# google-research/multinerf

Measured on NVIDIA H100. Metric: train-step rays/sec @16384 rays x (64+64+32) samples, higher is better.
Workload: dtype bf16

## Files before the change

multinerf_b200/csrc/chain.cu:

```cuda
#include <stdlib.h>
#include <string.h>

#include <algorithm>

#include "tc_common.cuh"

namespace mnrf {

constexpr int CH_W = 256;
constexpr int CH_ROWS = 128;
constexpr int CH_KBLK = CH_ROWS * 128;
constexpr int CH_WBLK = CH_W * 128;
constexpr int CH_SLOT = CH_WBLK + CH_KBLK;
constexpr int CH_SLOTS = 3;
constexpr int CH_ACT = 4 * CH_KBLK;
constexpr int CH_THREADS = 384;
constexpr int CH_MAX_LAYERS = MNRF_CHAIN_MAX_LAYERS;
constexpr int CH_SMEM = CH_ACT + CH_SLOTS * CH_SLOT + CH_MAX_LAYERS * CH_W * 4  + 256  +
                        1024 ;
static_assert(CH_SMEM <= 232448, "shared memory budget");

struct alignas(64) ChainMaps {
  CUtensorMap stream;
  CUtensorMap w[CH_MAX_LAYERS];
  CUtensorMap out[CH_MAX_LAYERS];
};

struct ChainLayer {
  int n_stream, stream_col0, stream_kb0;
  int n_res, res_kb0;
  int store;
  const float* bias;
  uint32_t* maskbits;
  int64_t ldmaskbits;
  float* colsum;
};

struct ChainParams {
  int num_layers;
  int64_t m;
  int64_t num_units;
  ChainLayer layer[CH_MAX_LAYERS];
  const float* head_w;
  const float* head_b;
  float* head_out;
};

__device__ __forceinline__ uint32_t pack_bf16_relu(float lo, float hi) {
  uint32_t r;
  asm("cvt.rn.relu.bf16x2.f32 %0, %1, %2;" : "=r"(r) : "f"(hi), "f"(lo));
  return r;
}

template <int MODE, int NH>
__global__ void __launch_bounds__(CH_THREADS, 1)
mlp_chain_kernel(const __grid_constant__ ChainMaps maps, const ChainParams p) {
  extern __shared__ uint8_t smem_dyn[];
  uint8_t* smem = reinterpret_cast<uint8_t*>((reinterpret_cast<uintptr_t>(smem_dyn) + 1023) & ~uintptr_t(1023));
  uint8_t* act = smem;
  uint8_t* ring = smem + CH_ACT;
  float* cs_s = reinterpret_cast<float*>(ring + CH_SLOTS * CH_SLOT);
  uint64_t* full_bar = reinterpret_cast<uint64_t*>(cs_s + CH_MAX_LAYERS * CH_W);
  uint64_t* empty_bar = full_bar + CH_SLOTS;

  const int warp = threadIdx.x >> 5;
  const int lane = threadIdx.x & 31;
  const int wg = threadIdx.x >> 7;

  if (threadIdx.x == 0) {
    bool any_stream = false;
    for (int j = 0; j < p.num_layers; ++j) {
      prefetch_tmap(&maps.w[j]);
      if (p.layer[j].store) prefetch_tmap(&maps.out[j]);
      any_stream |= p.layer[j].n_stream > 0;
    }
    if (any_stream) prefetch_tmap(&maps.stream);
    for (int i = 0; i < CH_SLOTS; ++i) { mbar_init(&full_bar[i], 1); mbar_init(&empty_bar[i], 8); }
    fence_barrier_init();
  }
  if (MODE == 1)
    for (int i = threadIdx.x; i < CH_MAX_LAYERS * CH_W; i += CH_THREADS) cs_s[i] = 0.f;
  __syncthreads();
  pdl_launch_dependents();
  pdl_wait();

  if (wg == 0) {
    setmaxnreg_dec<40>();
    if (threadIdx.x == 0) {
      uint32_t slot = 0, phase = 0;
      for (int64_t unit = blockIdx.x; unit < p.num_units; unit += gridDim.x) {
        const int row0 = (int)(unit * CH_ROWS);
        for (int j = 0; j < p.num_layers; ++j) {
          const ChainLayer& L = p.layer[j];
          for (int s = 0; s < L.n_res + L.n_stream; ++s) {
            const bool streamed = s >= L.n_res;
            const int si = s - L.n_res;
            mbar_wait(&empty_bar[slot], phase ^ 1, 1);
            mbar_expect_tx(&full_bar[slot], streamed ? CH_SLOT : CH_WBLK);
            uint8_t* sl = ring + slot * CH_SLOT;
            const int kb = streamed ? L.stream_kb0 + si : L.res_kb0 + s;
            tma_load_2d(sl, &maps.w[j], &full_bar[slot], kb * 64, 0);
            if (streamed) tma_load_2d(sl + CH_WBLK, &maps.stream, &full_bar[slot], L.stream_col0 + si * 64, row0);
            if (++slot == CH_SLOTS) { slot = 0; phase ^= 1; }
          }
        }
      }
    }
  } else {
    setmaxnreg_inc<232>();
    const int c = wg - 1;
    const int w = warp & 3;
    const int r_in = 64 * c + 16 * w + (lane >> 2);
    const int cq = 2 * (lane & 3);
    const uint32_t ring_s = smem_u32(ring), act_s = smem_u32(act);
    const bool lead = (threadIdx.x & 127) == 0;
    uint32_t slot = 0, phase = 0;
    float acc[CH_W / 2];
    for (int64_t unit = blockIdx.x; unit < p.num_units; unit += gridDim.x) {
      for (int j = 0; j < p.num_layers; ++j) {
        const ChainLayer& L = p.layer[j];
        const bool last = (j == p.num_layers - 1);
        const bool do_head = (MODE == 0) && last && p.head_w != nullptr;
        int prev = -1;
        fence_acc(acc);
        for (int s = 0; s < L.n_res + L.n_stream; ++s) {
          const bool streamed = s >= L.n_res;
          mbar_wait(&full_bar[slot], phase, 3);
          const uint32_t sl = ring_s + slot * CH_SLOT;
          const uint32_t a0 = (streamed ? sl + CH_WBLK : act_s + s * CH_KBLK) + c * (64 * 128);
          wgmma_fence();
#pragma unroll
          for (int k = 0; k < 64 / WGMMA_K; ++k)
            Wgmma<CH_W, 0, 0>::mma(acc, make_smem_desc(a0 + k * (WGMMA_K * 2), 0, 1024),
                                   make_smem_desc(sl + k * (WGMMA_K * 2), 0, 1024), (s > 0 || k > 0) ? 1u : 0u);
          wgmma_commit();
          wgmma_wait<1>();
          if (prev >= 0 && lane == 0) mbar_arrive(&empty_bar[prev]);
          prev = (int)slot;
          if (++slot == CH_SLOTS) { slot = 0; phase ^= 1; }
        }
        wgmma_wait<0>();
        fence_acc(acc);
        if (prev >= 0 && lane == 0) mbar_arrive(&empty_bar[prev]);

        if (lead) tma_store_wait_read<0>();
        named_bar_sync(1 + c, 128);
        int64_t rows[2];
        bool row_ok[2];
#pragma unroll
        for (int h = 0; h < 2; ++h) {
          rows[h] = unit * CH_ROWS + r_in + 8 * h;
          row_ok[h] = rows[h] < p.m;
        }
        uint32_t bits[2] = {0u, 0u};
        float hdot[NH][2];
#pragma unroll
        for (int o = 0; o < NH; ++o) hdot[o][0] = hdot[o][1] = 0.f;
#pragma unroll
        for (int i = 0; i < CH_W / 8; ++i) {
          const int col = 8 * i + cq;
          float v[2][2];
#pragma unroll
          for (int h = 0; h < 2; ++h) { v[h][0] = acc[4 * i + 2 * h]; v[h][1] = acc[4 * i + 2 * h + 1]; }
          uint32_t o[2];
          if (MODE == 0) {
            const float2 b = __ldg(reinterpret_cast<const float2*>(L.bias + col));
#pragma unroll
            for (int h = 0; h < 2; ++h) {
              v[h][0] += b.x;
              v[h][1] += b.y;
              bits[h] |= ((v[h][0] > 0.f ? 1u : 0u) | (v[h][1] > 0.f ? 2u : 0u)) << (col & 31);
              o[h] = pack_bf16_relu(v[h][0], v[h][1]);
            }
            if (do_head) {
#pragma unroll
              for (int oo = 0; oo < NH; ++oo) {
                const float2 hw = __ldg(reinterpret_cast<const float2*>(p.head_w + oo * CH_W + col));
#pragma unroll
                for (int h = 0; h < 2; ++h) hdot[oo][h] += bf16_lo(o[h]) * hw.x + bf16_hi(o[h]) * hw.y;
              }
            }
          } else {
#pragma unroll
            for (int h = 0; h < 2; ++h) {
              if (L.maskbits) {
                const uint32_t wd = row_ok[h] ? __ldg(L.maskbits + rows[h] * L.ldmaskbits + (col >> 5)) : 0u;
                if (!((wd >> (col & 31)) & 1u)) v[h][0] = 0.f;
                if (!((wd >> ((col + 1) & 31)) & 1u)) v[h][1] = 0.f;
              }
              o[h] = pack_bf16(v[h][0], v[h][1]);
            }
            if (L.colsum) {
              float s0 = v[0][0] + v[1][0], s1 = v[0][1] + v[1][1];
#pragma unroll
              for (int sh = 4; sh < 32; sh <<= 1) {
                s0 += __shfl_xor_sync(0xffffffffu, s0, sh);
                s1 += __shfl_xor_sync(0xffffffffu, s1, sh);
              }
              if (lane < 4) { atomicAdd(cs_s + j * CH_W + col, s0); atomicAdd(cs_s + j * CH_W + col + 1, s1); }
            }
          }
#pragma unroll
          for (int h = 0; h < 2; ++h) {
            const int r = r_in + 8 * h;
            st_shared_u32(act_s + (col >> 6) * CH_KBLK + r * 128 + ((((col & 63) >> 3) ^ (r & 7)) << 4) + (cq << 1), o[h]);
          }
          if (MODE == 0 && (i & 3) == 3) {
#pragma unroll
            for (int h = 0; h < 2; ++h) {
              bits[h] |= __shfl_xor_sync(0xffffffffu, bits[h], 1);
              bits[h] |= __shfl_xor_sync(0xffffffffu, bits[h], 2);
              if (L.maskbits && row_ok[h] && (lane & 3) == ((i >> 2) & 3))
                L.maskbits[rows[h] * L.ldmaskbits + (col >> 5)] = bits[h];
              bits[h] = 0u;
            }
          }
        }
        fence_proxy_async();
        named_bar_sync(1 + c, 128);
        if (lead && L.store) {
#pragma unroll
          for (int kb = 0; kb < 4; ++kb)
            tma_store_2d(&maps.out[j], act + kb * CH_KBLK + c * (64 * 128), kb * 64, (int)(unit * CH_ROWS) + 64 * c);
          tma_store_commit();
        }
        if (do_head) {
#pragma unroll
          for (int oo = 0; oo < NH; ++oo)
#pragma unroll
            for (int h = 0; h < 2; ++h) {
              hdot[oo][h] += __shfl_xor_sync(0xffffffffu, hdot[oo][h], 1);
              hdot[oo][h] += __shfl_xor_sync(0xffffffffu, hdot[oo][h], 2);
              if ((lane & 3) == 0 && row_ok[h])
                p.head_out[rows[h] * NH + oo] = hdot[oo][h] + (p.head_b ? __ldg(p.head_b + oo) : 0.f);
            }
        }
      }
    }
    if (lead) tma_store_wait_all();
    if (MODE == 1) {
      named_bar_sync(3, 256);
      for (int jj = 0; jj < p.num_layers; ++jj) {
        if (!p.layer[jj].colsum) continue;
        for (int i = threadIdx.x - 128; i < CH_W; i += 256) atomicAdd(p.layer[jj].colsum + i, cs_s[jj * CH_W + i]);
      }
    }
  }
}

}

extern "C" int mnrf_mlp_chain_max_layers(void) { return mnrf::CH_MAX_LAYERS; }

extern "C" int mnrf_mlp_chain(const mnrf_chain_desc* d, mnrf_stream stream_) {
  using namespace mnrf;
  cudaStream_t stream = (cudaStream_t)stream_;
  MNRF_CHECK(d, "mnrf_mlp_chain: null descriptor");
  if (d->m == 0) return 0;
  MNRF_CHECK(d->mode == MNRF_CHAIN_FWD || d->mode == MNRF_CHAIN_BWD, "mnrf_mlp_chain: bad mode %d", d->mode);
  MNRF_CHECK(d->num_layers >= 1 && d->num_layers <= CH_MAX_LAYERS, "mnrf_mlp_chain: 1..%d layers, got %d",
             CH_MAX_LAYERS, d->num_layers);
  MNRF_CHECK(d->width == CH_W, "mnrf_mlp_chain: layer width must be %d, got %d", CH_W, d->width);
  const int sms = mnrf_num_sms();
  ChainMaps maps;
  memset(&maps, 0, sizeof(maps));
  ChainParams p{};
  p.num_layers = d->num_layers;
  p.m = d->m;
  p.num_units = (d->m + CH_ROWS - 1) / CH_ROWS;
  bool any_stream = false;
  for (int j = 0; j < d->num_layers; ++j) {
    const mnrf_chain_layer& s = d->layer[j];
    ChainLayer& L = p.layer[j];
    MNRF_CHECK(s.n_res == 0 || s.n_res == CH_W / 64, "mnrf_mlp_chain: layer %d: n_res must be 0 or %d", j, CH_W / 64);
    MNRF_CHECK(s.n_stream >= 0 && (s.n_stream > 0 || s.n_res > 0), "mnrf_mlp_chain: layer %d has no operand", j);
    MNRF_CHECK(j > 0 || s.n_res == 0, "mnrf_mlp_chain: the first layer has no resident operand");
    MNRF_CHECK(s.w && ((uintptr_t)s.w % 16) == 0 && s.ldw % 8 == 0, "mnrf_mlp_chain: layer %d: weights must be 16-byte aligned", j);
    const int kblocks = std::max(s.n_stream > 0 ? s.stream_kb0 + s.n_stream : 0, s.n_res > 0 ? s.res_kb0 + s.n_res : 0);
    MNRF_CHECK(s.ldw >= (int64_t)kblocks * 64, "mnrf_mlp_chain: layer %d: weight pitch %lld < K %d", j, (long long)s.ldw, kblocks * 64);
    L.n_stream = s.n_stream; L.stream_col0 = s.stream_col0; L.stream_kb0 = s.stream_kb0;
    L.n_res = s.n_res; L.res_kb0 = s.res_kb0;
    L.store = s.out ? 1 : 0;
    L.bias = s.bias; L.maskbits = s.maskbits; L.ldmaskbits = s.ldmaskbits; L.colsum = s.colsum;
    if (s.bias) MNRF_CHECK(((uintptr_t)s.bias % 8) == 0, "mnrf_mlp_chain: layer %d: bias must be 8-byte aligned", j);
    if (s.maskbits)
      MNRF_CHECK(s.ldmaskbits >= CH_W / 32, "mnrf_mlp_chain: layer %d: maskbits rows must hold >= %d words", j, CH_W / 32);
    if (d->mode == MNRF_CHAIN_BWD) MNRF_CHECK(!s.bias, "mnrf_mlp_chain: bias is a forward input");
    else MNRF_CHECK(s.bias && !s.colsum, "mnrf_mlp_chain: layer %d: the forward chain takes a bias and no colsum", j);
    if (make_tmap(&maps.w[j], s.w, CH_W, (int64_t)kblocks * 64, s.ldw, 64, CH_W)) return 1;
    if (s.out) {
      MNRF_CHECK(((uintptr_t)s.out % 16) == 0 && s.ldo % 8 == 0 && s.ldo >= CH_W, "mnrf_mlp_chain: layer %d: output alignment", j);
      if (make_tmap(&maps.out[j], s.out, d->m, CH_W, s.ldo, 64, 64)) return 1;
    }
    any_stream |= s.n_stream > 0;
    if (s.n_stream > 0)
      MNRF_CHECK(s.stream_col0 % 64 == 0 && s.stream_col0 + s.n_stream * 64 <= d->stream_cols,
                 "mnrf_mlp_chain: layer %d: streamed columns [%d, %d) outside the stream tensor (%d columns)", j,
                 s.stream_col0, s.stream_col0 + s.n_stream * 64, d->stream_cols);
  }
  if (any_stream) {
    MNRF_CHECK(d->stream && ((uintptr_t)d->stream % 16) == 0 && d->ldstream % 8 == 0 && d->stream_cols % 64 == 0,
               "mnrf_mlp_chain: streamed operand must be 16-byte aligned with a multiple of 64 columns");
    if (make_tmap(&maps.stream, d->stream, d->m, d->stream_cols, d->ldstream, 64, CH_ROWS)) return 1;
  }
  p.head_w = d->head_w; p.head_b = d->head_b; p.head_out = d->head_out;
  const int head_n = d->head_n ? d->head_n : 1;
  if (d->head_w) MNRF_CHECK(d->mode == MNRF_CHAIN_FWD && d->head_out && ((uintptr_t)d->head_w % 16) == 0,
                            "mnrf_mlp_chain: the head is a forward output (16-byte aligned weights)");
  MNRF_CHECK(head_n == 1 || (head_n == 4 && d->head_w), "mnrf_mlp_chain: head_n must be 1 or 4, got %d", head_n);
  cudaLaunchConfig_t cfg = {};
  cfg.gridDim = dim3((unsigned)std::min<int64_t>(p.num_units, sms)); cfg.blockDim = dim3(CH_THREADS);
  cfg.dynamicSmemBytes = CH_SMEM; cfg.stream = stream;
  cudaLaunchAttribute attr[1];
  attr[0].id = cudaLaunchAttributeProgrammaticStreamSerialization;
  attr[0].val.programmaticStreamSerializationAllowed = 1;
  cfg.attrs = attr; cfg.numAttrs = pdl_enabled() ? 1 : 0;
  if (d->mode == MNRF_CHAIN_FWD && head_n == 4) {
    static bool set4 = false;
    auto kern = mlp_chain_kernel<0, 4>;
    if (!set4) { MNRF_CUDA(cudaFuncSetAttribute(kern, cudaFuncAttributeMaxDynamicSharedMemorySize, CH_SMEM)); set4 = true; }
    MNRF_CUDA(cudaLaunchKernelEx(&cfg, kern, maps, p));
  } else if (d->mode == MNRF_CHAIN_FWD) {
    static bool set0 = false;
    auto kern = mlp_chain_kernel<0, 1>;
    if (!set0) { MNRF_CUDA(cudaFuncSetAttribute(kern, cudaFuncAttributeMaxDynamicSharedMemorySize, CH_SMEM)); set0 = true; }
    MNRF_CUDA(cudaLaunchKernelEx(&cfg, kern, maps, p));
  } else {
    static bool set1 = false;
    auto kern = mlp_chain_kernel<1, 1>;
    if (!set1) { MNRF_CUDA(cudaFuncSetAttribute(kern, cudaFuncAttributeMaxDynamicSharedMemorySize, CH_SMEM)); set1 = true; }
    MNRF_CUDA(cudaLaunchKernelEx(&cfg, kern, maps, p));
  }
  MNRF_LAUNCH_CHECK();
  return 0;
}
```

Measured before the change: 187,100.

## Split chain MLP into N-halves to overlap epilogue with next wgmma

Each layer's 256-wide output is split into two 128-column halves, each with its own accumulator. The hi half's MMAs and the next layer's lead-in are issued while the lo half's epilogue runs, so tensor-core work overlaps the bias/ReLU/mask epilogue. The ring now holds single-operand stages (7 of them), and the activations are triple-buffered across 6 blocks. Streamed inputs are reloaded for each half, which doubles their TMA traffic. A clock-based stuck detector that traps on deadlock is also added.

```diff
diff --git a/multinerf_b200/csrc/chain.cu b/multinerf_b200/csrc/chain.cu
--- a/multinerf_b200/csrc/chain.cu
+++ b/multinerf_b200/csrc/chain.cu
@@ -8,17 +8,19 @@
 namespace mnrf {
 
 constexpr int CH_W = 256;
+constexpr int CH_HALF = CH_W / 2;
 constexpr int CH_ROWS = 128;
 constexpr int CH_KBLK = CH_ROWS * 128;
-constexpr int CH_WBLK = CH_W * 128;
-constexpr int CH_SLOT = CH_WBLK + CH_KBLK;
-constexpr int CH_SLOTS = 3;
-constexpr int CH_ACT = 4 * CH_KBLK;
+constexpr int CH_STAGE = CH_HALF * 128;
+static_assert(CH_STAGE == CH_KBLK, "a ring stage holds either operand");
+constexpr int CH_STAGES = 7;
+constexpr int CH_ACT_BUFS = 6;
 constexpr int CH_THREADS = 384;
 constexpr int CH_MAX_LAYERS = MNRF_CHAIN_MAX_LAYERS;
-constexpr int CH_SMEM = CH_ACT + CH_SLOTS * CH_SLOT + CH_MAX_LAYERS * CH_W * 4  + 256  +
-                        1024 ;
+constexpr int CH_SMEM = CH_ACT_BUFS * CH_KBLK + CH_STAGES * CH_STAGE + CH_MAX_LAYERS * CH_W * 4  +
+                        256  + 1024 ;
 static_assert(CH_SMEM <= 232448, "shared memory budget");
+static_assert(2 * CH_STAGES * 8 <= 256, "barrier space");
 
 struct alignas(64) ChainMaps {
   CUtensorMap stream;
@@ -52,16 +54,198 @@
   return r;
 }
 
+struct ChainRing {
+  uint32_t ring_s;
+  uint64_t* full_bar;
+  uint64_t* empty_bar;
+  uint32_t iss, rel;
+  bool stuck;
+
+  __device__ __forceinline__ uint32_t take() {
+    const uint32_t st = iss++;
+    uint64_t* bar = &full_bar[st % CH_STAGES];
+    const uint32_t parity = (st / CH_STAGES) & 1u;
+    if (!mbar_try_wait(bar, parity)) {
+      const long long t0 = clock64();
+      while (!stuck && !mbar_try_wait(bar, parity)) stuck = clock64() - t0 > 4000000000LL;
+    }
+    return ring_s + (st % CH_STAGES) * CH_STAGE;
+  }
+  __device__ __forceinline__ void release(uint32_t upto, int lane) {
+    for (; rel < upto; ++rel)
+      if (lane == 0) mbar_arrive(&empty_bar[rel % CH_STAGES]);
+  }
+};
+
+__device__ __forceinline__ void chain_issue(float (&acc)[64], const ChainLayer& L, int q0, int q1, ChainRing& R,
+                                            uint32_t act_s, int prev, int c) {
+  for (int q = q0; q < q1; ++q) {
+    uint32_t a0;
+    if (q < L.n_res) a0 = act_s + ((prev + q) % CH_ACT_BUFS) * CH_KBLK;
+    else a0 = R.take();
+    a0 += c * (64 * 128);
+    const uint32_t w0 = R.take();
+    wgmma_fence();
+#pragma unroll
+    for (int k = 0; k < 64 / WGMMA_K; ++k)
+      Wgmma<CH_HALF, 0, 0>::mma(acc, make_smem_desc(a0 + k * (WGMMA_K * 2), 0, 1024),
+                                make_smem_desc(w0 + k * (WGMMA_K * 2), 0, 1024), (q > 0 || k > 0) ? 1u : 0u);
+  }
+}
+
+__device__ __forceinline__ void chain_rest(float (&acc)[64], const ChainLayer& L, int q0, ChainRing& R,
+                                           uint32_t act_s, int prev, int c, int lane) {
+  for (int q = q0; q < L.n_res + L.n_stream; ++q) {
+    const uint32_t first = R.iss;
+    chain_issue(acc, L, q, q + 1, R, act_s, prev, c);
+    wgmma_commit();
+    wgmma_wait<1>();
+    R.release(first, lane);
+  }
+}
+
+__device__ __forceinline__ int chain_fit(const ChainLayer& L, int cap, const ChainRing& R) {
+  int room = CH_STAGES - (int)(R.iss - R.rel), n = 0;
+  for (; n < cap && n < L.n_res + L.n_stream; ++n) {
+    room -= n < L.n_res ? 1 : 2;
+    if (room < 0) break;
+  }
+  return n;
+}
+
+__device__ __forceinline__ void chain_lead_in(float (&acc)[64], const ChainLayer& L, int n, ChainRing& R,
+                                              uint32_t act_s, int prev, int c, int lane) {
+  const uint32_t first = R.iss;
+  fence_acc(acc);
+  chain_issue(acc, L, 0, n, R, act_s, prev, c);
+  wgmma_commit();
+  wgmma_wait<1>();
+  R.release(first, lane);
+}
+
+struct ChainRows {
+  int64_t unit;
+  int64_t rows[2];
+  bool row_ok[2];
+};
+
+template <int MODE, int NH, int H>
+__device__ __forceinline__ void chain_epilogue(const float (&acc)[64], const ChainParams& p, const ChainMaps& maps,
+                                               int j, const ChainRows& rw, float (&hdot)[NH][2], uint32_t act_s,
+                                               uint8_t* act, int cur, float* cs_s, int c, int r_in, int cq,
+                                               int lane, bool lead) {
+  const ChainLayer& L = p.layer[j];
+  const bool do_head = (MODE == 0) && j == p.num_layers - 1 && p.head_w != nullptr;
+  const int b0 = (cur + 2 * H) % CH_ACT_BUFS, b1 = (cur + 2 * H + 1) % CH_ACT_BUFS;
+  uint32_t mw[2][4];
+  if (MODE == 1) {
+#pragma unroll
+    for (int h = 0; h < 2; ++h)
+#pragma unroll
+      for (int wd = 0; wd < 4; ++wd)
+        mw[h][wd] = L.maskbits && rw.row_ok[h] ? __ldg(L.maskbits + rw.rows[h] * L.ldmaskbits + 4 * H + wd) : 0u;
+  }
+  if (lead) tma_store_wait_read<2>();
+  named_bar_sync(1 + c, 128);
+  uint32_t bits[2] = {0u, 0u};
+  if (H == 0) {
+#pragma unroll
+    for (int o = 0; o < NH; ++o) hdot[o][0] = hdot[o][1] = 0.f;
+  }
+#pragma unroll
+  for (int i = 0; i < CH_HALF / 8; ++i) {
+    const int col = CH_HALF * H + 8 * i + cq;
+    float v[2][2];
+#pragma unroll
+    for (int h = 0; h < 2; ++h) { v[h][0] = acc[4 * i + 2 * h]; v[h][1] = acc[4 * i + 2 * h + 1]; }
+    uint32_t o[2];
+    if (MODE == 0) {
+      const float2 b = __ldg(reinterpret_cast<const float2*>(L.bias + col));
+#pragma unroll
+      for (int h = 0; h < 2; ++h) {
+        v[h][0] += b.x;
+        v[h][1] += b.y;
+        bits[h] |= ((v[h][0] > 0.f ? 1u : 0u) | (v[h][1] > 0.f ? 2u : 0u)) << (col & 31);
+        o[h] = pack_bf16_relu(v[h][0], v[h][1]);
+      }
+      if (do_head) {
+#pragma unroll
+        for (int oo = 0; oo < NH; ++oo) {
+          const float2 hw = __ldg(reinterpret_cast<const float2*>(p.head_w + oo * CH_W + col));
+#pragma unroll
+          for (int h = 0; h < 2; ++h) hdot[oo][h] += bf16_lo(o[h]) * hw.x + bf16_hi(o[h]) * hw.y;
+        }
+      }
+    } else {
+#pragma unroll
+      for (int h = 0; h < 2; ++h) {
+        if (L.maskbits) {
+          const uint32_t wd = mw[h][i >> 2];
+          if (!((wd >> (col & 31)) & 1u)) v[h][0] = 0.f;
+          if (!((wd >> ((col + 1) & 31)) & 1u)) v[h][1] = 0.f;
+        }
+        o[h] = pack_bf16(v[h][0], v[h][1]);
+      }
+      if (L.colsum) {
+        float s0 = v[0][0] + v[1][0], s1 = v[0][1] + v[1][1];
+#pragma unroll
+        for (int sh = 4; sh < 32; sh <<= 1) {
+          s0 += __shfl_xor_sync(0xffffffffu, s0, sh);
+          s1 += __shfl_xor_sync(0xffffffffu, s1, sh);
+        }
+        if (lane < 4) { atomicAdd(cs_s + j * CH_W + col, s0); atomicAdd(cs_s + j * CH_W + col + 1, s1); }
+      }
+    }
+    const uint32_t blk = act_s + (i < 8 ? b0 : b1) * CH_KBLK;
+#pragma unroll
+    for (int h = 0; h < 2; ++h) {
+      const int r = r_in + 8 * h;
+      st_shared_u32(blk + r * 128 + ((((col & 63) >> 3) ^ (r & 7)) << 4) + (cq << 1), o[h]);
+    }
+    if (MODE == 0 && (i & 3) == 3) {
+#pragma unroll
+      for (int h = 0; h < 2; ++h) {
+        bits[h] |= __shfl_xor_sync(0xffffffffu, bits[h], 1);
+        bits[h] |= __shfl_xor_sync(0xffffffffu, bits[h], 2);
+        if (L.maskbits && rw.row_ok[h] && (lane & 3) == ((i >> 2) & 3))
+          L.maskbits[rw.rows[h] * L.ldmaskbits + (col >> 5)] = bits[h];
+        bits[h] = 0u;
+      }
+    }
+  }
+  fence_proxy_async();
+  named_bar_sync(1 + c, 128);
+  if (lead) {
+    if (L.store) {
+      const int row0 = (int)(rw.unit * CH_ROWS) + 64 * c;
+      tma_store_2d(&maps.out[j], act + b0 * CH_KBLK + c * (64 * 128), (2 * H) * 64, row0);
+      tma_store_2d(&maps.out[j], act + b1 * CH_KBLK + c * (64 * 128), (2 * H + 1) * 64, row0);
+    }
+    tma_store_commit();
+  }
+  if (H == 1 && do_head) {
+#pragma unroll
+    for (int oo = 0; oo < NH; ++oo)
+#pragma unroll
+      for (int h = 0; h < 2; ++h) {
+        hdot[oo][h] += __shfl_xor_sync(0xffffffffu, hdot[oo][h], 1);
+        hdot[oo][h] += __shfl_xor_sync(0xffffffffu, hdot[oo][h], 2);
+        if ((lane & 3) == 0 && rw.row_ok[h])
+          p.head_out[rw.rows[h] * NH + oo] = hdot[oo][h] + (p.head_b ? __ldg(p.head_b + oo) : 0.f);
+      }
+  }
+}
+
 template <int MODE, int NH>
 __global__ void __launch_bounds__(CH_THREADS, 1)
 mlp_chain_kernel(const __grid_constant__ ChainMaps maps, const ChainParams p) {
   extern __shared__ uint8_t smem_dyn[];
   uint8_t* smem = reinterpret_cast<uint8_t*>((reinterpret_cast<uintptr_t>(smem_dyn) + 1023) & ~uintptr_t(1023));
   uint8_t* act = smem;
-  uint8_t* ring = smem + CH_ACT;
-  float* cs_s = reinterpret_cast<float*>(ring + CH_SLOTS * CH_SLOT);
+  uint8_t* ring = smem + CH_ACT_BUFS * CH_KBLK;
+  float* cs_s = reinterpret_cast<float*>(ring + CH_STAGES * CH_STAGE);
   uint64_t* full_bar = reinterpret_cast<uint64_t*>(cs_s + CH_MAX_LAYERS * CH_W);
-  uint64_t* empty_bar = full_bar + CH_SLOTS;
+  uint64_t* empty_bar = full_bar + CH_STAGES;
 
   const int warp = threadIdx.x >> 5;
   const int lane = threadIdx.x & 31;
@@ -75,7 +259,7 @@
       any_stream |= p.layer[j].n_stream > 0;
     }
     if (any_stream) prefetch_tmap(&maps.stream);
-    for (int i = 0; i < CH_SLOTS; ++i) { mbar_init(&full_bar[i], 1); mbar_init(&empty_bar[i], 8); }
+    for (int i = 0; i < CH_STAGES; ++i) { mbar_init(&full_bar[i], 1); mbar_init(&empty_bar[i], 8); }
     fence_barrier_init();
   }
   if (MODE == 1)
@@ -87,22 +271,25 @@
   if (wg == 0) {
     setmaxnreg_dec<40>();
     if (threadIdx.x == 0) {
-      uint32_t slot = 0, phase = 0;
+      uint32_t st = 0;
+      auto load = [&](const CUtensorMap* map, int c0, int c1) {
+        const uint32_t s = st % CH_STAGES;
+        mbar_wait(&empty_bar[s], ((st / CH_STAGES) & 1u) ^ 1u, 1);
+        mbar_expect_tx(&full_bar[s], CH_STAGE);
+        tma_load_2d(ring + s * CH_STAGE, map, &full_bar[s], c0, c1);
+        ++st;
+      };
       for (int64_t unit = blockIdx.x; unit < p.num_units; unit += gridDim.x) {
         const int row0 = (int)(unit * CH_ROWS);
         for (int j = 0; j < p.num_layers; ++j) {
           const ChainLayer& L = p.layer[j];
-          for (int s = 0; s < L.n_res + L.n_stream; ++s) {
-            const bool streamed = s >= L.n_res;
-            const int si = s - L.n_res;
-            mbar_wait(&empty_bar[slot], phase ^ 1, 1);
-            mbar_expect_tx(&full_bar[slot], streamed ? CH_SLOT : CH_WBLK);
-            uint8_t* sl = ring + slot * CH_SLOT;
-            const int kb = streamed ? L.stream_kb0 + si : L.res_kb0 + s;
-            tma_load_2d(sl, &maps.w[j], &full_bar[slot], kb * 64, 0);
-            if (streamed) tma_load_2d(sl + CH_WBLK, &maps.stream, &full_bar[slot], L.stream_col0 + si * 64, row0);
-            if (++slot == CH_SLOTS) { slot = 0; phase ^= 1; }
-          }
+          for (int h = 0; h < 2; ++h)
+            for (int q = 0; q < L.n_res + L.n_stream; ++q) {
+              const bool streamed = q >= L.n_res;
+              const int si = q - L.n_res;
+              if (streamed) load(&maps.stream, L.stream_col0 + si * 64, row0);
+              load(&maps.w[j], (streamed ? L.stream_kb0 + si : L.res_kb0 + q) * 64, CH_HALF * h);
+            }
         }
       }
     }
@@ -112,131 +299,54 @@
     const int w = warp & 3;
     const int r_in = 64 * c + 16 * w + (lane >> 2);
     const int cq = 2 * (lane & 3);
-    const uint32_t ring_s = smem_u32(ring), act_s = smem_u32(act);
+    const uint32_t act_s = smem_u32(act);
     const bool lead = (threadIdx.x & 127) == 0;
-    uint32_t slot = 0, phase = 0;
-    float acc[CH_W / 2];
+    ChainRing R{smem_u32(ring), full_bar, empty_bar, 0u, 0u, false};
+    float acc_lo[CH_HALF / 2], acc_hi[CH_HALF / 2];
+    float hdot[NH][2];
+    int cur = 0;
+    int pre = 0;
+    if ((int64_t)blockIdx.x < p.num_units) {
+      pre = chain_fit(p.layer[0], 2, R);
+      fence_acc(acc_lo);
+      chain_issue(acc_lo, p.layer[0], 0, pre, R, act_s, 0, c);
+      wgmma_commit();
+    }
     for (int64_t unit = blockIdx.x; unit < p.num_units; unit += gridDim.x) {
+      ChainRows rw;
+      rw.unit = unit;
+#pragma unroll
+      for (int h = 0; h < 2; ++h) {
+        rw.rows[h] = unit * CH_ROWS + r_in + 8 * h;
+        rw.row_ok[h] = rw.rows[h] < p.m;
+      }
       for (int j = 0; j < p.num_layers; ++j) {
         const ChainLayer& L = p.layer[j];
-        const bool last = (j == p.num_layers - 1);
-        const bool do_head = (MODE == 0) && last && p.head_w != nullptr;
-        int prev = -1;
-        fence_acc(acc);
-        for (int s = 0; s < L.n_res + L.n_stream; ++s) {
-          const bool streamed = s >= L.n_res;
-          mbar_wait(&full_bar[slot], phase, 3);
-          const uint32_t sl = ring_s + slot * CH_SLOT;
-          const uint32_t a0 = (streamed ? sl + CH_WBLK : act_s + s * CH_KBLK) + c * (64 * 128);
-          wgmma_fence();
-#pragma unroll
-          for (int k = 0; k < 64 / WGMMA_K; ++k)
-            Wgmma<CH_W, 0, 0>::mma(acc, make_smem_desc(a0 + k * (WGMMA_K * 2), 0, 1024),
-                                   make_smem_desc(sl + k * (WGMMA_K * 2), 0, 1024), (s > 0 || k > 0) ? 1u : 0u);
-          wgmma_commit();
-          wgmma_wait<1>();
-          if (prev >= 0 && lane == 0) mbar_arrive(&empty_bar[prev]);
-          prev = (int)slot;
-          if (++slot == CH_SLOTS) { slot = 0; phase ^= 1; }
+        const int prev = (cur + 2) % CH_ACT_BUFS;
+        chain_rest(acc_lo, L, pre, R, act_s, prev, c, lane);
+        wgmma_wait<0>();
+        fence_acc(acc_lo);
+        R.release(R.iss, lane);
+        const int hi_pre = L.n_res > 0 ? L.n_res : (L.n_stream < 2 ? L.n_stream : 2);
+        fence_acc(acc_hi);
+        chain_issue(acc_hi, L, 0, hi_pre, R, act_s, prev, c);
+        wgmma_commit();
+        chain_epilogue<MODE, NH, 0>(acc_lo, p, maps, j, rw, hdot, act_s, act, cur, cs_s, c, r_in, cq, lane, lead);
+        chain_rest(acc_hi, L, hi_pre, R, act_s, prev, c, lane);
+        const int next = j + 1 < p.num_layers ? j + 1 : unit + gridDim.x < p.num_units ? 0 : -1;
+        if (next >= 0) {
+          pre = chain_fit(p.layer[next], 2, R);
+          chain_lead_in(acc_lo, p.layer[next], pre, R, act_s, cur, c, lane);
+        } else {
+          wgmma_wait<0>();
+          R.release(R.iss, lane);
         }
-        wgmma_wait<0>();
-        fence_acc(acc);
-        if (prev >= 0 && lane == 0) mbar_arrive(&empty_bar[prev]);
-
-        if (lead) tma_store_wait_read<0>();
-        named_bar_sync(1 + c, 128);
-        int64_t rows[2];
-        bool row_ok[2];
-#pragma unroll
-        for (int h = 0; h < 2; ++h) {
-          rows[h] = unit * CH_ROWS + r_in + 8 * h;
-          row_ok[h] = rows[h] < p.m;
-        }
-        uint32_t bits[2] = {0u, 0u};
-        float hdot[NH][2];
-#pragma unroll
-        for (int o = 0; o < NH; ++o) hdot[o][0] = hdot[o][1] = 0.f;
-#pragma unroll
-        for (int i = 0; i < CH_W / 8; ++i) {
-          const int col = 8 * i + cq;
-          float v[2][2];
-#pragma unroll
-          for (int h = 0; h < 2; ++h) { v[h][0] = acc[4 * i + 2 * h]; v[h][1] = acc[4 * i + 2 * h + 1]; }
-          uint32_t o[2];
-          if (MODE == 0) {
-            const float2 b = __ldg(reinterpret_cast<const float2*>(L.bias + col));
-#pragma unroll
-            for (int h = 0; h < 2; ++h) {
-              v[h][0] += b.x;
-              v[h][1] += b.y;
-              bits[h] |= ((v[h][0] > 0.f ? 1u : 0u) | (v[h][1] > 0.f ? 2u : 0u)) << (col & 31);
-              o[h] = pack_bf16_relu(v[h][0], v[h][1]);
-            }
-            if (do_head) {
-#pragma unroll
-              for (int oo = 0; oo < NH; ++oo) {
-                const float2 hw = __ldg(reinterpret_cast<const float2*>(p.head_w + oo * CH_W + col));
-#pragma unroll
-                for (int h = 0; h < 2; ++h) hdot[oo][h] += bf16_lo(o[h]) * hw.x + bf16_hi(o[h]) * hw.y;
-              }
-            }
-          } else {
-#pragma unroll
-            for (int h = 0; h < 2; ++h) {
-              if (L.maskbits) {
-                const uint32_t wd = row_ok[h] ? __ldg(L.maskbits + rows[h] * L.ldmaskbits + (col >> 5)) : 0u;
-                if (!((wd >> (col & 31)) & 1u)) v[h][0] = 0.f;
-                if (!((wd >> ((col + 1) & 31)) & 1u)) v[h][1] = 0.f;
-              }
-              o[h] = pack_bf16(v[h][0], v[h][1]);
-            }
-            if (L.colsum) {
-              float s0 = v[0][0] + v[1][0], s1 = v[0][1] + v[1][1];
-#pragma unroll
-              for (int sh = 4; sh < 32; sh <<= 1) {
-                s0 += __shfl_xor_sync(0xffffffffu, s0, sh);
-                s1 += __shfl_xor_sync(0xffffffffu, s1, sh);
-              }
-              if (lane < 4) { atomicAdd(cs_s + j * CH_W + col, s0); atomicAdd(cs_s + j * CH_W + col + 1, s1); }
-            }
-          }
-#pragma unroll
-          for (int h = 0; h < 2; ++h) {
-            const int r = r_in + 8 * h;
-            st_shared_u32(act_s + (col >> 6) * CH_KBLK + r * 128 + ((((col & 63) >> 3) ^ (r & 7)) << 4) + (cq << 1), o[h]);
-          }
-          if (MODE == 0 && (i & 3) == 3) {
-#pragma unroll
-            for (int h = 0; h < 2; ++h) {
-              bits[h] |= __shfl_xor_sync(0xffffffffu, bits[h], 1);
-              bits[h] |= __shfl_xor_sync(0xffffffffu, bits[h], 2);
-              if (L.maskbits && row_ok[h] && (lane & 3) == ((i >> 2) & 3))
-                L.maskbits[rows[h] * L.ldmaskbits + (col >> 5)] = bits[h];
-              bits[h] = 0u;
-            }
-          }
-        }
-        fence_proxy_async();
-        named_bar_sync(1 + c, 128);
-        if (lead && L.store) {
-#pragma unroll
-          for (int kb = 0; kb < 4; ++kb)
-            tma_store_2d(&maps.out[j], act + kb * CH_KBLK + c * (64 * 128), kb * 64, (int)(unit * CH_ROWS) + 64 * c);
-          tma_store_commit();
-        }
-        if (do_head) {
-#pragma unroll
-          for (int oo = 0; oo < NH; ++oo)
-#pragma unroll
-            for (int h = 0; h < 2; ++h) {
-              hdot[oo][h] += __shfl_xor_sync(0xffffffffu, hdot[oo][h], 1);
-              hdot[oo][h] += __shfl_xor_sync(0xffffffffu, hdot[oo][h], 2);
-              if ((lane & 3) == 0 && row_ok[h])
-                p.head_out[rows[h] * NH + oo] = hdot[oo][h] + (p.head_b ? __ldg(p.head_b + oo) : 0.f);
-            }
-        }
-      }
-    }
+        fence_acc(acc_hi);
+        chain_epilogue<MODE, NH, 1>(acc_hi, p, maps, j, rw, hdot, act_s, act, cur, cs_s, c, r_in, cq, lane, lead);
+        cur = (cur + 4) % CH_ACT_BUFS;
+      }
+    }
+    if (R.stuck) __trap();
     if (lead) tma_store_wait_all();
     if (MODE == 1) {
       named_bar_sync(3, 256);
@@ -287,7 +397,7 @@
       MNRF_CHECK(s.ldmaskbits >= CH_W / 32, "mnrf_mlp_chain: layer %d: maskbits rows must hold >= %d words", j, CH_W / 32);
     if (d->mode == MNRF_CHAIN_BWD) MNRF_CHECK(!s.bias, "mnrf_mlp_chain: bias is a forward input");
     else MNRF_CHECK(s.bias && !s.colsum, "mnrf_mlp_chain: layer %d: the forward chain takes a bias and no colsum", j);
-    if (make_tmap(&maps.w[j], s.w, CH_W, (int64_t)kblocks * 64, s.ldw, 64, CH_W)) return 1;
+    if (make_tmap(&maps.w[j], s.w, CH_W, (int64_t)kblocks * 64, s.ldw, 64, CH_HALF)) return 1;
     if (s.out) {
       MNRF_CHECK(((uintptr_t)s.out % 16) == 0 && s.ldo % 8 == 0 && s.ldo >= CH_W, "mnrf_mlp_chain: layer %d: output alignment", j);
       if (make_tmap(&maps.out[j], s.out, d->m, CH_W, s.ldo, 64, 64)) return 1;
```

Result: faster. 190,100, median of 6 (+1.6%).
